# kjyv/FloBaRoID

Hardware: AMD Instinct MI355X
Metric: regressor samples/s (fused regressor->Gram pass) + TSQR TFLOP/s, WALK-MAN 31-DOF float-base (higher is better)
Workload: dtype f64

## Files before the change

flobaroid_amd/csrc/fbr_gram64.h:

```cpp
#pragma once
#define FBR_G64_SWZ(c) (2 * ((c) & 15))
#include <algorithm>
#include <type_traits>
#include <utility>

#include "fbr_kinid.h"

struct FbrGram64Tile {
    int col[FBR_TILE];
    std::vector<int> path;
    int friction = 0;
    int lo = 0, hi = 0;
};

struct FbrGram64 {
    int NT = 0;
    int NF = 0;
    int nlev = 0, fb = 0, flev = 0, ntr = 0, maxact = 0, npw = 0, wpb = 8;
    long blk_doubles = 0;
    std::vector<int> trow;
    std::vector<int> slab;
    int nstage = 0, base_stages = 0;
    std::vector<int> stage_lev;
    std::vector<int> lev_begin;
// ... 510 lines not shown
        const long grp = blk / bpg, lb = blk - grp * bpg;
        const long base = grp * Sg + (lb << 6);
        const int valid = (int)min(64L, Sg - (lb << 6));
        __syncthreads();
        {
            const long off = base * n;
            const int cnt = valid * n;
            int sr = tid / n, dc = tid - sr * n;
            const int ds = nth / n, dd = nth - ds * n;
            for (int i = tid; i < cnt; i += nth) {
                const double a = q[off + i], b = dq[off + i], c = ddq[off + i];
                sq[sr * ldn + dc] = a;
                sdq[sr * ldn + dc] = b;
                sddq[sr * ldn + dc] = c;
                sr += ds;
                dc += dd;
                if (dc >= n) {
                    dc -= n;
                    sr++;
                }
            }
            if (HASW || wr.k) {
                const int cw = valid * rows;
                int wr_ = tid / rows, wc = tid - wr_ * rows;
                const int es = nth / rows, ed = nth - es * rows;
                for (int i = tid; i < cw; i += nth) {
                    const double wv = HASW ? wts[base * rows + i] : 1.0;
                    if (HASW) sw[wr_ * ldw + wc] = wv;
                    if constexpr (KR == 1) {
                        if (wr.k) st[wr_ * ldw + wc] = wv * wv * rhs[base * rows + i];
                    } else {
#pragma unroll
                        for (int r = 0; r < KR; r++) st[r * 64 * ldw + wr_ * ldw + wc] = wv * wv * rhs[(base * rows + i) * KR + r];
                    }
                    wr_ += es;
                    wc += ed;
                    if (wc >= rows) {
                        wc -= rows;
                        wr_++;
                    }
                }
            }
        }
        __syncthreads();
        const int ls = min(lane, valid - 1);
        const long s = base + ls;
        const bool live = lane < valid;
        const double *mysq = sq + ls * ldn, *mysdq = sdq + ls * ldn, *mysddq = sddq + ls * ldn, *myw = sw + ls * ldw, *myt = st + ls * ldw;
        const long slot_off = blk * blk_doubles + (long)(lane >> 5) * 512;
        const int s31 = lane & 31;
        auto state = [&](int d, double &a, double &b, double &c) {
            a = mysq[d];
            b = mysdq[d];
            c = mysddq[d];
        };
        auto basest = [&](double *v6, double *a6, double *e3) {
            for (int i = 0; i < 6; i++) {
                v6[i] = bv[s * 6 + i];
                a6[i] = ba[s * 6 + i];
            }
            for (int i = 0; i < 3; i++) e3[i] = rpy[s * 3 + i];
        };
        auto save = [&](int b, int i, double v) { scr[(b * FBR_LINK_REC + i) * 64] = v; };
        auto load = [&](int b, int i) { return scr[(b * FBR_LINK_REC + i) * 64]; };
        auto consts = [&](int l, double *rR, double *rp, double *ax) {
            const fbr_cdouble_ptr cR = (fbr_cdouble_ptr)(unsigned long)m.restR, cp = (fbr_cdouble_ptr)(unsigned long)m.restp,
                                  ca = (fbr_cdouble_ptr)(unsigned long)m.axis;
            for (int i = 0; i < 9; i++) rR[i] = cR[9 * l + i];
            for (int i = 0; i < 3; i++) {
                rp[i] = cp[3 * l + i];
                ax[i] = ca[3 * l + i];
            }
        };
        const unsigned vlane = (unsigned)(((unsigned long)slot_off + (unsigned long)s31) << 3);
        auto link = [&](int l, int depth, const double *rec, const double (*Sst)[6], const int *lvd, double *F) {
            (void)F;
            if (wr.base_only) depth = 0;
            __builtin_amdgcn_s_waitcnt(0x0F70);
            long d10[10], dF[4];
#pragma unroll
            for (int pp = 0; pp < 10; pp++) d10[pp] = cdst[((long)part * m.L + l) * FBR_G64_WORDS + pp];
#pragma unroll
            for (int pp = 0; pp < 4; pp++) dF[pp] = cdst[((long)part * m.L + l) * FBR_G64_WORDS + 10 + pp];
            auto ft_of = [&](int ro, double *F) {
#pragma unroll
                for (int i = 0; i < 6; i++)
                    if (i < m.fb) F[i] = myt[ro + i];
#pragma unroll
                for (int j = 0; j < MAXD; j++)
                    if (j < depth) {
                        const double tj = myt[ro + m.fb + lvd[j]];
#pragma unroll
                        for (int i = 0; i < 6; i++) F[i] += Sst[j][i] * tj;
                    }
            };
            double Ft[6] = {0.0, 0.0, 0.0, 0.0, 0.0, 0.0};
            if constexpr (KR == 1) {
                if (wr.k) {
#pragma unroll
                    for (int i = 0; i < 6; i++)
                        if (i < m.fb) Ft[i] = myt[i];
#pragma unroll
                    for (int j = 0; j < MAXD; j++)
                        if (j < depth) {
                            const double tj = myt[m.fb + lvd[j]];
#pragma unroll
                            for (int i = 0; i < 6; i++) Ft[i] += Sst[j][i] * tj;
                        }
                }
            }
            auto ft_group = [&](int r, double *F) {
                int ro = r * 64 * ldw;
                asm volatile("" : "+v"(ro));
#pragma unroll
                for (int i = 0; i < 6; i++) F[i] = 0.0;
                ft_of(ro, F);
            };
            auto store = [&](long d0, int lv, double v) {
                if (d0 == 0) return;
                const unsigned vo = vlane ^ ((unsigned)(d0 & 0xff) << 3);
                __builtin_nontemporal_store(v, (fbr_gdouble_ptr)((fbr_gchar_ptr)(d0 & ~0xffL) + (long)lv * 8192 + vo));
            };
            auto full_group = [&](auto q0c, auto nqc) {
                constexpr int Q0 = decltype(q0c)::value, NQ = decltype(nqc)::value;
                double wA[NQ][6];
#pragma unroll
                for (int qq = 0; qq < NQ; qq++) fbr_unit_wrench(rec, Q0 + qq, wA[qq]);
#pragma unroll
                for (int i = 0; i < 6; i++)
                    if (i < m.fb) {
#pragma unroll
                        for (int qq = 0; qq < NQ; qq++) store(i < wr.flev ? dF[Q0 + qq] : d10[Q0 + qq], i, HASW ? wA[qq][i] * myw[i] : wA[qq][i]);
                    }
#pragma unroll
                for (int j = 0; j < MAXD; j++)
                    if (j < depth) {
                        double v[NQ];
#pragma unroll
                        for (int qq = 0; qq < NQ; qq++) v[qq] = fbr_dot6(Sst[j], wA[qq]);
                        const double wj = HASW ? myw[m.fb + lvd[j]] : 1.0;
#pragma unroll
                        for (int qq = 0; qq < NQ; qq++) store(d10[Q0 + qq], m.fb + j, HASW ? v[qq] * wj : v[qq]);
                    }
                if constexpr (KR == 1) {
                    if (wr.k) {
#pragma unroll
                        for (int qq = 0; qq < NQ; qq++)
                            if (d10[Q0 + qq]) unsafeAtomicAdd(mo + (long)ccol[10 * l + Q0 + qq] * 64 + lane, fbr_dot6(Ft, wA[qq]));
                    }
                } else {
#pragma unroll
                    for (int r = 0; r < KR; r++) {
                        double F[6];
                        ft_group(r, F);
#pragma unroll
                        for (int qq = 0; qq < NQ; qq++)
                            if (d10[Q0 + qq]) unsafeAtomicAdd(mo + ((long)r * wr.cols + ccol[10 * l + Q0 + qq]) * 64 + lane, fbr_dot6(F, wA[qq]));
                    }
                }
            };
            auto moment_group = [&](auto q0c, auto nqc) {
                constexpr int Q0 = decltype(q0c)::value, NQ = decltype(nqc)::value;
                double nB[NQ][3];
#pragma unroll
                for (int qq = 0; qq < NQ; qq++) fbr_unit_moment3(rec, 4 + Q0 + qq, nB[qq]);
#pragma unroll
                for (int i = 3; i < 6; i++)
                    if (i < m.fb) {
#pragma unroll
                        for (int qq = 0; qq < NQ; qq++) store(d10[4 + Q0 + qq], i, HASW ? nB[qq][i - 3] * myw[i] : nB[qq][i - 3]);
                    }
#pragma unroll
                for (int j = 0; j < MAXD; j++)
                    if (j < depth) {
                        double v[NQ];
#pragma unroll
                        for (int qq = 0; qq < NQ; qq++) v[qq] = Sst[j][3] * nB[qq][0] + Sst[j][4] * nB[qq][1] + Sst[j][5] * nB[qq][2];
                        const double wj = HASW ? myw[m.fb + lvd[j]] : 1.0;
#pragma unroll
                        for (int qq = 0; qq < NQ; qq++) store(d10[4 + Q0 + qq], m.fb + j, HASW ? v[qq] * wj : v[qq]);
                    }
                if constexpr (KR == 1) {
                    if (wr.k) {
#pragma unroll
                        for (int qq = 0; qq < NQ; qq++)
                            if (d10[4 + Q0 + qq])
                                unsafeAtomicAdd(mo + (long)ccol[10 * l + 4 + Q0 + qq] * 64 + lane, Ft[3] * nB[qq][0] + Ft[4] * nB[qq][1] + Ft[5] * nB[qq][2]);
                    }
                } else {
#pragma unroll
                    for (int r = 0; r < KR; r++) {
                        double F[6];
                        ft_group(r, F);
#pragma unroll
                        for (int qq = 0; qq < NQ; qq++)
                            if (d10[4 + Q0 + qq])
                                unsafeAtomicAdd(mo + ((long)r * wr.cols + ccol[10 * l + 4 + Q0 + qq]) * 64 + lane,
                                                F[3] * nB[qq][0] + F[4] * nB[qq][1] + F[5] * nB[qq][2]);
                    }
                }
            };
            using std::integral_constant;
            if constexpr (MAXD > 8 && MAXD <= 10) {
                full_group(integral_constant<int, 0>{}, integral_constant<int, 2>{});
                full_group(integral_constant<int, 2>{}, integral_constant<int, 2>{});
                moment_group(integral_constant<int, 0>{}, integral_constant<int, 3>{});
                moment_group(integral_constant<int, 3>{}, integral_constant<int, 3>{});
            } else {
                full_group(integral_constant<int, 0>{}, integral_constant<int, 4>{});
                moment_group(integral_constant<int, 0>{}, integral_constant<int, 6>{});
            }
            const int nfr = wr.cols > wr.ninert ? (wr.cols - wr.ninert) / n : 0;
            const int dj = nfr ? m.dof[l] : -1;
            if (dj >= 0 && depth > 0) {
                const fbr_cint_ptr cfr = (fbr_cint_ptr)(unsigned long)(wr.lcol10 + (long)wr.nparts * 10 * m.L + ((long)part * m.L + l) * FBR_G64_FRIC);
#pragma unroll
                for (int pf = 0; pf < FBR_G64_FRIC; pf++)
                    if (pf < nfr) {
                        const long dfw = cdst[((long)part * m.L + l) * FBR_G64_WORDS + 14 + pf];
                        if (dfw == 0) continue;
                        const int c = cfr[pf];
                        const double fv = fbr_friction_value(m.coldesc[c].z, mysdq[dj], sign ? sign[s * n + dj] : 0.0, m.stribeck);
                        store(dfw, m.fb + depth - 1, HASW ? fv * myw[m.fb + dj] : fv);
                        if constexpr (KR == 1) {
                            if (wr.k) unsafeAtomicAdd(mo + (long)c * 64 + lane, fv * myt[m.fb + dj]);
                        } else {
#pragma unroll
                            for (int r = 0; r < KR; r++) unsafeAtomicAdd(mo + ((long)r * wr.cols + c) * 64 + lane, fv * myt[r * 64 * ldw + m.fb + dj]);
                        }
                    }
            }
        };
        auto emit = [&](int, double) {};
        if (live) {
            fbr_kinid_lane<MAXD, false>(wr.part_nsteps[part], p.maxlvl, p.steps + wr.part_step0[part] * FBR_KINID_STEP, p.endflush, m.floating, m.g, m.fb,
                                        state, basest, save, load, link, emit, consts);
            if constexpr (KR == 1) {
                if (wr.k && part == wr.nparts - 1) {
                    double tt = 0.0;
                    for (int r = 0; r < rows; r++) {
                        const double wv = HASW ? myw[r] : 1.0, tv = rhs[s * rows + r] * wv;
                        tt += tv * tv;
                    }
                    unsafeAtomicAdd(mo + (long)wr.cols * 64 + lane, tt);
                }
            } else if (part == wr.nparts - 1) {
                double tt[KR * (KR + 1) / 2];
#pragma unroll
                for (int e = 0; e < KR * (KR + 1) / 2; e++) tt[e] = 0.0;
                for (int r = 0; r < rows; r++) {
                    const double wv = HASW ? myw[r] : 1.0;
                    double tv[KR];
#pragma unroll
                    for (int i = 0; i < KR; i++) tv[i] = rhs[(s * rows + r) * KR + i] * wv;
#pragma unroll
                    for (int i = 0, e = 0; i < KR; i++)
#pragma unroll
                        for (int j = i; j < KR; j++, e++) tt[e] += tv[i] * tv[j];
                }
#pragma unroll
                for (int e = 0; e < KR * (KR + 1) / 2; e++) unsafeAtomicAdd(mo + ((long)KR * wr.cols + e) * 64 + lane, tt[e]);
            }
        }
    }
}

__global__ __launch_bounds__(256) void fbr_gram64_tail_zero_kernel(double *__restrict__ img, long blk_doubles, long bpg, int ntr, int valid)
{
    double *blk = img + ((long)blockIdx.y * bpg + bpg - 1) * blk_doubles;
    const int per = 16 * (64 - valid);
    for (long e = (long)blockIdx.x * blockDim.x + threadIdx.x; e < (long)ntr * per; e += (long)gridDim.x * blockDim.x) {
        const int tr = (int)(e / per), r = (int)(e - (long)tr * per), c = r / (64 - valid), sl = valid + r % (64 - valid);
        blk[(long)tr * 1024 + (sl >> 5) * 512 + c * 32 + ((sl & 31) ^ FBR_G64_SWZ(c))] = 0.0;
    }
}

__global__ __launch_bounds__(256) void fbr_gram64_mom_reduce_kernel(int P, int k, int nwg, const double *__restrict__ mom, double *__restrict__ G)
{
    __shared__ double part[256];
    const int c = blockIdx.x, t = threadIdx.x, nm = fbr_gram64_mom_count(P, k);
    double s0 = 0.0, s1 = 0.0, s2 = 0.0, s3 = 0.0;
    int i = t;
    for (; i + 768 < nwg * 64; i += 1024) {
        s0 += mom[((long)(i >> 6) * nm + c) * 64 + (i & 63)];
        s1 += mom[((long)((i + 256) >> 6) * nm + c) * 64 + ((i + 256) & 63)];
        s2 += mom[((long)((i + 512) >> 6) * nm + c) * 64 + ((i + 512) & 63)];
        s3 += mom[((long)((i + 768) >> 6) * nm + c) * 64 + ((i + 768) & 63)];
    }
    for (; i < nwg * 64; i += 256) s0 += mom[((long)(i >> 6) * nm + c) * 64 + (i & 63)];
    part[t] = (s0 + s1) + (s2 + s3);
    __syncthreads();
    for (int o = 128; o > 0; o >>= 1) {
        if (t < o) part[t] += part[t + o];
        __syncthreads();
    }
    if (t) return;
    const int Pa = P + k;
    int row, col;
    fbr_gram64_mom_target(P, k, c, &row, &col);
    G[(long)row * Pa + col] += part[0];
    if (row != col) G[(long)col * Pa + row] += part[0];
}

template <int NPW, int WPB, bool RUNS = false>
__global__ __launch_bounds__(WPB * 64, (NPW <= 10) ? 4 : 2) void fbr_gram64_kernel(DevGram64 g, long nblk, const double *__restrict__ img,
                                                                                  double *__restrict__ partial, int carry)
{
    constexpr int MW = 3 * NPW;
    static_assert(MW <= 64, "a wave's slot table is fetched with one load");
    extern __shared__ __attribute__((aligned(16))) double smem[];
    const int bufd = g.maxact * 512;
    double *buf0 = smem, *buf1 = smem + bufd;
    int *slab = (int *)(smem + 2 * bufd);
    int *levb = slab + g.nlev * g.NT;
    int *pcs = levb + g.nlev + 1;
    int *wm = pcs + 2 * g.npieces;
    int *rn = wm + WPB * MW;
    static_assert(!RUNS || NPW > 10, "the 128-register shapes walk every slot");
    int *stl = rn + (RUNS ? WPB * g.nlev : 0);
    const int tid = threadIdx.x, lane = tid & 63;
    const int wave = __builtin_amdgcn_readfirstlane(tid >> 6);
    for (int i = tid; i < g.nlev * g.NT; i += WPB * 64) slab[i] = g.slab[i] * 512;
    for (int i = tid; i <= g.nlev; i += WPB * 64) levb[i] = g.lev_begin[i];
    for (int i = tid; i < 2 * g.npieces; i += WPB * 64) pcs[i] = g.pieces[i];
    for (int i = tid; i < WPB * MW; i += WPB * 64) wm[i] = g.wmeta[i];
    if (RUNS)
        for (int i = tid; i < WPB * g.nlev; i += WPB * 64) rn[i] = g.runs[i];
    for (int i = tid; i <= g.nstage; i += WPB * 64) stl[i] = g.stage_lev[i];
    fbr_d4 acc[NPW];
    img += (long)blockIdx.y * nblk * g.blk_doubles;
    double *pp = partial + (((((long)blockIdx.y * gridDim.x + blockIdx.x) * 8 + (wave & 7)) * (WPB / 8) + (wave >> 3)) * NPW) * 256;
    if (carry) {
#pragma unroll
        for (int q = 0; q < NPW; q++) acc[q] = (fbr_d4){pp[q * 256 + lane], pp[q * 256 + 64 + lane], pp[q * 256 + 128 + lane], pp[q * 256 + 192 + lane]};
    } else {
#pragma unroll
        for (int q = 0; q < NPW; q++) acc[q] = (fbr_d4){0.0, 0.0, 0.0, 0.0};
    }
    __syncthreads();
    const int nmine = (int)((nblk - blockIdx.x + gridDim.x - 1) / gridDim.x);
    const long nst = (long)(nmine > 0 ? nmine : 0) * 2 * g.nstage;
    const int svl = stl[lane <= g.nstage ? lane : 0], svp = levb[svl];
    auto dma = [&](int sg, long bh, int par) {
        const long blk = (long)blockIdx.x + (bh >> 1) * gridDim.x;
        const double *src = img + blk * g.blk_doubles + (bh & 1) * 512 + 2 * lane;
        double *buf = par ? buf1 : buf0;
        const int i0 = __builtin_amdgcn_readlane(svp, sg) + wave, i1 = __builtin_amdgcn_readlane(svp, sg + 1);
        const int mine = i0 < i1 ? (i1 - i0 + WPB - 1) / WPB : 0;
        const int il = i0 + (lane < mine ? lane : 0) * WPB;
        const int gxv = mine > 0 ? pcs[2 * il] : 0, lxv = mine > 0 ? pcs[2 * il + 1] : 0;
        for (int j = 0; j < mine; j++) {
            const int gx = __builtin_amdgcn_readlane(gxv, j), lx = __builtin_amdgcn_readlane(lxv, j);
            __builtin_amdgcn_global_load_lds((fbr_glb_ptr)(src + gx), (fbr_lds_ptr)(buf + lx), 16, 0, 0);
        }
    };
    if (nst > 0) dma(0, 0, 0);
    const int li = lane & 15, kk = lane >> 4;
    const int lofs = li * 32, sx = FBR_G64_SWZ(li);
    const int mv = wm[wave * MW + (lane < MW ? lane : 0)];
    const int idxv = (lane < MW && (lane % 3) != 2 && mv >= 0) ? mv : 0;
    const int p0c = lofs | (sx ^ kk);
    static_assert(!RUNS || MW < 63, "lane 63 holds the run");
    const int *lk = lane == 63 ? rn + wave * g.nlev : slab + idxv;
    const int lks = lane == 63 ? 1 : g.NT;
    const unsigned rlm = [&] {
        unsigned m = 0;
#pragma unroll
        for (int q = 1; q < NPW; q++) m |= (unsigned)(__builtin_amdgcn_readlane(mv, 3 * q) != __builtin_amdgcn_readlane(mv, 3 * q - 3)) << q;
        return (unsigned)__builtin_amdgcn_readfirstlane((int)m);
    }();
    int ko[8];
#pragma unroll
    for (int ks = 0; ks < 8; ks++) ko[ks] = (p0c ^ (4 * ks)) * 8;
    double X[2][8], Y[2][8];
#pragma unroll
    for (int ks = 0; ks < 8; ks++) X[0][ks] = X[1][ks] = Y[0][ks] = Y[1][ks] = 0.0;
    auto run_stage = [&](const double *buf, int lv0, int lv1) {
        const unsigned bufb = (unsigned)(unsigned long)(fbr_lds_ptr)buf;
        int offv = lk[lv0 * lks];
        for (int lv = lv0; lv < lv1; lv++) {
            const int cur = offv;
            offv = lk[(lv + 1 < g.nlev ? lv + 1 : lv) * lks];
            const int run = __builtin_amdgcn_readlane(cur, 63), qa = run & 0xff, qb = run >> 8;
#define G64_RD(D, S, K, T) "v_add_u32 %[" T "], %[" S "], %[o" #K "]\n\tds_read_b64 %[" D #K "], %[" T "]\n\t"
#define G64_MF(K) "v_mfma_f64_16x16x4_f64 %[acc], %[xa" #K "], %[xb" #K "], %[acc]\n\t"
#define G64_MV(K) "v_mov_b64 %[ya" #K "], %[xa" #K "]\n\t"
#pragma unroll
            for (int q = 0; q < NPW; q++) {
                if (q < qa || q >= qb) continue;
                const int P = q & 1, N = P ^ 1;
                int t0, t1;
                if (q == qa) {
                    const unsigned sa = bufb + (__builtin_amdgcn_readlane(cur, 3 * q) << 3), sb = bufb + (__builtin_amdgcn_readlane(cur, 3 * q + 1) << 3);
                    asm volatile(G64_RD("xa", "sa", 0, "t0") G64_RD("xa", "sa", 1, "t1") G64_RD("xa", "sa", 2, "t0") G64_RD("xa", "sa", 3, "t1")
                                 G64_RD("xa", "sa", 4, "t0") G64_RD("xa", "sa", 5, "t1") G64_RD("xa", "sa", 6, "t0") G64_RD("xa", "sa", 7, "t1")
                                 G64_RD("xb", "sb", 0, "t0") G64_RD("xb", "sb", 1, "t1") G64_RD("xb", "sb", 2, "t0") G64_RD("xb", "sb", 3, "t1")
                                 G64_RD("xb", "sb", 4, "t0") G64_RD("xb", "sb", 5, "t1") G64_RD("xb", "sb", 6, "t0") G64_RD("xb", "sb", 7, "t1")
                                 : [t0] "=&v"(t0), [t1] "=&v"(t1),
                                   [xa0] "+v"(X[P][0]), [xa1] "+v"(X[P][1]), [xa2] "+v"(X[P][2]), [xa3] "+v"(X[P][3]),
                                   [xa4] "+v"(X[P][4]), [xa5] "+v"(X[P][5]), [xa6] "+v"(X[P][6]), [xa7] "+v"(X[P][7]),
                                   [xb0] "+v"(Y[P][0]), [xb1] "+v"(Y[P][1]), [xb2] "+v"(Y[P][2]), [xb3] "+v"(Y[P][3]),
                                   [xb4] "+v"(Y[P][4]), [xb5] "+v"(Y[P][5]), [xb6] "+v"(Y[P][6]), [xb7] "+v"(Y[P][7])
                                 : [sa] "s"(sa), [sb] "s"(sb),
                                   [o0] "v"(ko[0]), [o1] "v"(ko[1]), [o2] "v"(ko[2]), [o3] "v"(ko[3]), [o4] "v"(ko[4]), [o5] "v"(ko[5]), [o6] "v"(ko[6]), [o7] "v"(ko[7])
                                 : "memory");
                }
                const int f = __builtin_amdgcn_readfirstlane((q + 1 < qb ? 4 : 0) | ((rlm >> (q + 1)) & 1 ? 8 : 0));
                const unsigned sna = q + 1 < NPW ? bufb + (__builtin_amdgcn_readlane(cur, 3 * q + 3) << 3) : 0u;
                const unsigned snb = q + 1 < NPW ? bufb + (__builtin_amdgcn_readlane(cur, 3 * q + 4) << 3) : 0u;
                asm volatile(
                    "s_waitcnt lgkmcnt(0)\n\t"
                    G64_MF(0)
                    "s_bitcmp0_b32 %[f], 2\n\t"
                    "s_cbranch_scc1 3f\n\t"
                    G64_RD("yb", "snb", 0, "t0") G64_RD("yb", "snb", 1, "t1") G64_MF(1)
                    G64_RD("yb", "snb", 2, "t0") G64_RD("yb", "snb", 3, "t1") G64_MF(2)
                    G64_RD("yb", "snb", 4, "t0") G64_RD("yb", "snb", 5, "t1") G64_MF(3)
                    G64_RD("yb", "snb", 6, "t0") G64_RD("yb", "snb", 7, "t1") G64_MF(4)
                    "s_bitcmp0_b32 %[f], 3\n\t"
                    "s_cbranch_scc1 2f\n\t"
                    G64_RD("ya", "sna", 0, "t0") G64_RD("ya", "sna", 1, "t1") G64_RD("ya", "sna", 2, "t0") G64_RD("ya", "sna", 3, "t1") G64_MF(5)
                    G64_RD("ya", "sna", 4, "t0") G64_RD("ya", "sna", 5, "t1") G64_RD("ya", "sna", 6, "t0") G64_RD("ya", "sna", 7, "t1") G64_MF(6)
                    G64_MF(7)
                    "s_branch 9f\n\t"
                    "2:\n\t"
                    G64_MV(0) G64_MV(1) G64_MV(2) G64_MV(3) G64_MF(5)
                    G64_MV(4) G64_MV(5) G64_MV(6) G64_MV(7) G64_MF(6)
                    G64_MF(7)
                    "s_branch 9f\n\t"
                    "3:\n\t"
                    G64_MF(1) G64_MF(2) G64_MF(3) G64_MF(4) G64_MF(5) G64_MF(6) G64_MF(7)
                    "9:"
                    : [acc] "+v"(acc[q]), [t0] "=&v"(t0), [t1] "=&v"(t1),
                      [xa0] "+v"(X[P][0]), [xa1] "+v"(X[P][1]), [xa2] "+v"(X[P][2]), [xa3] "+v"(X[P][3]),
                      [xa4] "+v"(X[P][4]), [xa5] "+v"(X[P][5]), [xa6] "+v"(X[P][6]), [xa7] "+v"(X[P][7]),
                      [xb0] "+v"(Y[P][0]), [xb1] "+v"(Y[P][1]), [xb2] "+v"(Y[P][2]), [xb3] "+v"(Y[P][3]),
                      [xb4] "+v"(Y[P][4]), [xb5] "+v"(Y[P][5]), [xb6] "+v"(Y[P][6]), [xb7] "+v"(Y[P][7]),
                      [ya0] "+v"(X[N][0]), [ya1] "+v"(X[N][1]), [ya2] "+v"(X[N][2]), [ya3] "+v"(X[N][3]),
                      [ya4] "+v"(X[N][4]), [ya5] "+v"(X[N][5]), [ya6] "+v"(X[N][6]), [ya7] "+v"(X[N][7]),
                      [yb0] "+v"(Y[N][0]), [yb1] "+v"(Y[N][1]), [yb2] "+v"(Y[N][2]), [yb3] "+v"(Y[N][3]),
                      [yb4] "+v"(Y[N][4]), [yb5] "+v"(Y[N][5]), [yb6] "+v"(Y[N][6]), [yb7] "+v"(Y[N][7])
                    : [f] "s"(f), [sna] "s"(sna), [snb] "s"(snb),
                      [o0] "v"(ko[0]), [o1] "v"(ko[1]), [o2] "v"(ko[2]), [o3] "v"(ko[3]), [o4] "v"(ko[4]), [o5] "v"(ko[5]), [o6] "v"(ko[6]), [o7] "v"(ko[7])
                    : "memory", "scc");
            }
#undef G64_RD
#undef G64_MF
#undef G64_MV
        }
    };
    int sg = 0;
    long bh = 0;
    for (long st = 0; st < nst; st++) {
        asm volatile("s_waitcnt vmcnt(0)" ::: "memory");
        __syncthreads();
        const int sgn = sg + 1 == g.nstage ? 0 : sg + 1;
        const long bhn = sgn ? bh : bh + 1;
        if (st + 1 < nst) dma(sgn, bhn, (int)((st + 1) & 1));
        const double *buf = (st & 1) ? buf1 : buf0;
        const int lv0 = __builtin_amdgcn_readlane(svl, sg), lv1 = __builtin_amdgcn_readlane(svl, sg + 1);
        sg = sgn;
        bh = bhn;
        if constexpr (RUNS) {
            run_stage(buf, lv0, lv1);
            continue;
        }
        for (int lv = lv0; lv < lv1; lv++) {
            const int offv = slab[lv * g.NT + idxv];
            int curI = -1;
            double a[8] = {0.0, 0.0, 0.0, 0.0, 0.0, 0.0, 0.0, 0.0};
#pragma unroll
            for (int q = 0; q < NPW; q++) {
                const int tI = __builtin_amdgcn_readlane(mv, 3 * q), rg = __builtin_amdgcn_readlane(mv, 3 * q + 2);
                if (tI < 0 || lv < (rg & 0xff) || lv >= (rg >> 8)) continue;
                const double *pb = buf + __builtin_amdgcn_readlane(offv, 3 * q + 1);
                double b[NPW <= 10 ? 4 : 8];
                int p0 = p0c;
                if constexpr (NPW <= 10) asm volatile("" : "+v"(p0));
                if (tI != curI) {
                    const double *pa = buf + __builtin_amdgcn_readlane(offv, 3 * q);
#pragma unroll
                    for (int ks = 0; ks < 8; ks++) a[ks] = pa[p0 ^ (4 * ks)];
                    curI = tI;
                }
                constexpr int KG = NPW <= 10 ? 4 : 8;
#pragma unroll
                for (int k0 = 0; k0 < 8; k0 += KG) {
#pragma unroll
                    for (int ks = k0; ks < k0 + KG; ks++) b[ks - k0] = pb[p0 ^ (4 * ks)];
                    __builtin_amdgcn_sched_barrier(0);
#pragma unroll
                    for (int ks = k0; ks < k0 + KG; ks++) acc[q] = __builtin_amdgcn_mfma_f64_16x16x4f64(a[ks], b[ks - k0], acc[q], 0, 0, 0);
                    __builtin_amdgcn_sched_barrier(0);
                }
            }
        }
    }
    if constexpr (RUNS) asm volatile("s_nop 7\n\ts_nop 7\n\ts_nop 7" ::: "memory");
#pragma unroll
    for (int q = 0; q < NPW; q++) {
        pp[q * 256 + 0 * 64 + lane] = acc[q][0];
        pp[q * 256 + 1 * 64 + lane] = acc[q][1];
        pp[q * 256 + 2 * 64 + lane] = acc[q][2];
        pp[q * 256 + 3 * 64 + lane] = acc[q][3];
    }
}
#endif
```

flobaroid_amd/csrc/fbr_gram_api.hip:

```cpp
#define FBR_KERNELS_GRAM
#include "fbr_internal.h"

static int get_deal(GramHolder *h, int wpg, GramHolder::Deal *out, bool base_only = false)
{
    const int key = wpg | (base_only ? 1 << 24 : 0);
    auto it = h->deals.find(key);
    if (it != h->deals.end()) {
        *out = it->second;
        return FBR_OK;
    }
    const std::vector<int> n = fbr_gram_deal(h->prog, wpg, base_only);
    std::vector<int2> tab;
    std::vector<int> begin(h->prog.T + 1, 0), given(h->prog.T, 0);
    for (int p = 0; p < h->prog.T; p++) begin[p + 1] = begin[p] + n[p];
    while ((int)tab.size() < begin[h->prog.T])
        for (int p = 0; p < h->prog.T; p++)
            if (given[p] < n[p]) tab.push_back(make_int2(p, given[p]++ | (n[p] << 16)));
    GramHolder::Deal d;
    int rc;
    if ((rc = upload(h->pool, tab, &d.tab))) return rc;
    if ((rc = upload(h->pool, begin, &d.begin))) return rc;
    h->deals[key] = d;
    *out = d;
    return FBR_OK;
// ... 663 lines not shown
            fresh_images = true;
        }
    HIPCHK(hipEventRecord(m->ev_fork, m->stream));
    hipStream_t side = m->opt.gram_serial ? m->stream : m->side;
    const bool cross = overlap_prev && !fresh_images && side != m->stream;
    if (!cross) HIPCHK(hipStreamWaitEvent(side, m->ev_fork, 0));
    if (h2d_chunked && (rc = ensure_stage_buffers(m, d, k, dw, ch, nchunks > 1 ? 2 : 1))) return rc;
    const int pack_wgs_per_cu = 24;
    const int pack_blocks_max = m->num_cus * pack_wgs_per_cu;
    auto produce = [&](long ci) -> int {
        const long s0 = items[ci].s0, cs = items[ci].cs;
        const int b = (int)(ci & 1);
        if (ci >= 2 || (cross && m->ev_gram_rec[b])) HIPCHK(hipStreamWaitEvent(side, m->ev_gram[b], 0));
        DevStates dc = d;
        long o = s0;
        const double *crhs = drhs, *cw = dw;
        if (h2d_chunked) {
            int r3;
            if ((r3 = ensure_copy_stream(m))) return r3;
            if (ci >= 2 || (cross && m->ev_pack_rec[b]))
                HIPCHK(hipStreamWaitEvent(m->copy, m->ev_pack[b], 0));
            else
                HIPCHK(hipStreamWaitEvent(m->copy, m->ev_fork, 0));
            ProfScope ps(m, FBR_PROF_H2D, m->copy);
            if ((r3 = stage_chunk(m, d, drhs, k, dw, s0, cs, b, m->copy, &dc, &crhs, &cw))) return r3;
            o = 0;
            HIPCHK(hipEventRecord(m->ev_h2d[b], m->copy));
            HIPCHK(hipStreamWaitEvent(side, m->ev_h2d[b], 0));
        }
        int rc2 = run_kin(m, dc, o, cs, side, &m->rec2);
        if (rc2) return rc2;
        {
            ProfScope ps(m, FBR_PROF_PACK, side);
            const int blocks = (int)std::min<long>(cs, (long)pack_blocks_max);
            hipLaunchKernelGGL(fbr_pack_kernel, dim3(blocks), dim3(256), h->pack_lds_bytes, side, h->dev, m->dm, cs, cs / items[ci].ng,
                               m->rec2.as<double>(), dc.dq + o * hm.n, dc.sign ? dc.sign + o * hm.n : nullptr,
                               crhs ? crhs + (size_t)o * hm.rows * k : nullptr, cw ? cw + (size_t)o * hm.rows : nullptr,
                               h->pimg[b].as<double>(), base_only ? 1 : 0, moments ? h->mom[(int)(m->next_ticket & 1)].as<double>() : nullptr);
        }
        HIPCHK(hipGetLastError());
        HIPCHK(hipEventRecord(m->ev_pack[b], side));
        m->ev_pack_rec[b] = true;
        return FBR_OK;
    };
    const int mpar = (int)(m->next_ticket & 1);
    if (moments) {
        const size_t mbytes = (size_t)pack_blocks_max * 256 * 4 * sizeof(double);
        if (h->mom[mpar].bytes < mbytes) h->mom_clean[mpar] = false;
        if ((rc = h->mom[mpar].ensure(mbytes))) return rc;
        if (!h->mom_clean[mpar]) HIPCHK(hipMemsetAsync(h->mom[mpar].p, 0, mbytes, side));
        h->mom_clean[mpar] = false;
    }
    if ((rc = produce(0))) return rc;
    for (long ci = 0; ci < nchunks; ci++) {
        const long cs = items[ci].cs;
        const int ng = items[ci].ng;
        const int b = (int)(ci & 1);
        if (ci + 1 < nchunks && (rc = produce(ci + 1))) return rc;
        HIPCHK(hipStreamWaitEvent(m->stream, m->ev_pack[b], 0));
        const int wpg = wpg_of(cs, ng);
        GramHolder::Deal deal;
        if ((rc = get_deal(h, wpg, &deal, base_only))) return rc;
        DevGram dg = h->dev;
        dg.wpg = wpg;
        dg.ks_limit = base_only ? hm.fbp / 4 : (1 << 20);
        if (base_only && hm.fbp == 8) {
            dg.pieces = dg.pieces_b;
            dg.piece_begin = dg.piece_begin_b;
        }
        dg.wg_tab = deal.tab;
        dg.wg_begin = deal.begin;
        const int NW = wpg * ng;
        const size_t pcount = (size_t)NW * FBR_WPB * FBR_NPW * 256;
        if ((rc = m->partial.ensure(pcount * sizeof(double)))) return rc;
        unsigned long long *dbg = nullptr;
        if (timing) {
            if ((rc = m->st_x.ensure((size_t)NW * FBR_WPB * 8 * sizeof(unsigned long long)))) return rc;
            dbg = m->st_x.as<unsigned long long>();
        }
        {
            ProfScope ps(m, FBR_PROF_GRAM);
            hipLaunchKernelGGL(gram_kernel, dim3(NW), dim3(FBR_WPB * 64), h->lds_bytes, m->stream, dg, cs, ng,
                               h->pimg[b].as<double>(), m->partial.as<double>(), dbg, (carry_ok && ci > 0) ? 1 : 0);
        }
        HIPCHK(hipGetLastError());
        HIPCHK(hipEventRecord(m->ev_gram[b], m->stream));
        m->ev_gram_rec[b] = true;
        if (timing && (rc = print_gram_timing(m, T, dbg, NW))) return rc;
        if (!carry_ok || ci + 1 == nchunks) {
            ProfScope ps(m, FBR_PROF_REDUCE);
            hipLaunchKernelGGL(fbr_gram_reduce_kernel, dim3(T * FBR_WPB * FBR_NPW, ng), dim3(256), 0, m->stream, dg,
                               m->partial.as<double>(), G + (size_t)items[ci].g0 * Pa * Pa);
        }
        HIPCHK(hipGetLastError());
    }
    if (moments) {
        ProfScope ps(m, FBR_PROF_REDUCE);
        hipLaunchKernelGGL(fbr_gram_mom_reduce_kernel, dim3(256), dim3(256), 0, m->stream, hm.cols, k, pack_blocks_max, h->itemcol,
                           h->mom[mpar].as<double>(), G);
        HIPCHK(hipGetLastError());
        h->mom_clean[mpar] = true;
    }
    if (!async) HIPCHK(hipStreamSynchronize(side));
    return FBR_OK;
}

static int gram_impl_inner(fbr_model *m, const fbr_states *st, const double *rhs, int32_t k, const double *w, double *G_out,
                           int32_t out_mem, int32_t accumulate, int32_t ngroups, int64_t *async_ticket)
{
    const bool async = async_ticket != nullptr;
    bool overlap_prev = false;
    const bool h2d_chunked = st && st->mem == FBR_HOST && m && m->opt.h2d_chunked && is_pinned_host(st->q) && is_pinned_host(st->dq) &&
                             is_pinned_host(st->ddq) && is_pinned_host(st->base_vel) && is_pinned_host(st->base_acc) &&
                             is_pinned_host(st->base_rpy) && is_pinned_host(st->sign) && is_pinned_host(rhs) && is_pinned_host(w);
    if (async && (!st || out_mem != FBR_DEVICE || (st->mem != FBR_DEVICE && !h2d_chunked))) {
        set_err("fbr_gram_submit takes a device-resident output and device-resident or PINNED host states / rhs / weights");
        return FBR_E_INVALID;
    }
    DevStates d;
    if (m) m->submitting = async;
    int rc = stage_states(m, st, &d, true, h2d_chunked);
    if (m) m->submitting = false;
    if (rc) return rc;
    if (async) {
        if ((rc = wait_ticket(m, m->next_ticket - 2))) return rc;
        overlap_prev = m->waited_ticket < m->next_ticket - 1;
    }
    if (!G_out || k < 0 || k > FBR_MAX_RHS || (k > 0 && !rhs)) {
        set_err("bad rhs / G_out arguments");
        return FBR_E_INVALID;
    }
    if (ngroups < 1 || d.S % ngroups != 0) {
        set_err("the number of samples must be a multiple of the number of groups");
        return FBR_E_INVALID;
    }
    const FbrHostModel &hm = m->hm;
    if ((hm.rows + 3) / 4 * 4 > 60) {
        if (async || ngroups != 1) {
            set_err("robots with more than 60 regressor rows per sample (54 DOF on a floating base) are served by the blocking, ungrouped "
                    "fbr_gram_accumulate only (Gram from the TSQR factor): fbr_gram_submit / fbr_gram_grouped are limited to 60 rows");
            return FBR_E_UNSUPPORTED;
        }
        return gram_via_tsqr(m, st, rhs, k, w, G_out, out_mem, accumulate);
    }
    GramHolder *h = nullptr;
    const bool moments = ngroups == 1 && fbr_gram_rhs_moments(hm, k, m->opt.gram_rhs_tile != 0) && !m->opt.gram_timing;
    if ((rc = get_gram(m, k, &h, moments))) return rc;
    const int Pa = h->prog.Pa;
    const size_t gcount = (size_t)Pa * Pa * ngroups;
    const long S = d.S;
    const double *drhs = nullptr, *dw = nullptr;
    if (h2d_chunked) {
        drhs = rhs;
        dw = w;
    } else {
        if ((rc = stage_one(m, m->st_aux, rhs, (size_t)S * hm.rows * k, st->mem, &drhs))) return rc;
        if ((rc = stage_one(m, m->st_aux2, w, (size_t)S * hm.rows, st->mem, &dw))) return rc;
    }
    bool base_only = false;
    if (w && S > 0 && hm.fb > 0 && hm.rows > hm.fb) {
        if (st->mem == FBR_HOST) {
            base_only = true;
            for (long s = 0; s < S && base_only; s++)
                for (int r = hm.fb; r < hm.rows; r++)
                    if (w[s * hm.rows + r] != 0.0) {
                        base_only = false;
                        break;
                    }
        } else {
            std::vector<char> act;
            if ((rc = active_rows(m, dw, S, &act))) return rc;
            base_only = true;
            for (int r = hm.fb; r < hm.rows; r++) base_only = base_only && !act[r];
        }
    }
    double *G = G_out;
    if (out_mem == FBR_HOST) {
        if ((rc = m->g_tmp.ensure(gcount * sizeof(double)))) return rc;
        G = m->g_tmp.as<double>();
        if (accumulate) HIPCHK(hipMemcpyAsync(G, G_out, gcount * sizeof(double), hipMemcpyHostToDevice, m->stream));
    }
    if (!accumulate) HIPCHK(hipMemsetAsync(G, 0, gcount * sizeof(double), m->stream));
    bool lane = false;
    if (S > 0 && d.q && !m->opt.gram_timing && !m->opt.gram_serial && (ngroups == 1 || (k == 0 && !h2d_chunked && !base_only)) &&
        (rc = gram64_serves(m, h, k, &lane)))
        return rc;
    if (lane && ngroups > 1 && (S / ngroups + 63) / 64 <= gram64_chunk_blocks(h->g64))
        rc = gram64_grouped_pass(m, h, d, dw, G, ngroups);
    else if (lane && ngroups == 1)
        rc = gram64_pass(m, h, d, drhs, dw, k, G, base_only && h->g64.base_stages > 0, h2d_chunked);
    else if (S > 0)
        rc = gram_image_pass(m, h, d, drhs, dw, k, G, ngroups, base_only, h2d_chunked, overlap_prev, async);
    if (rc) return rc;
    if (S > 0 && !async && h2d_chunked && m->copy) HIPCHK(hipStreamSynchronize(m->copy));
    if (async) {
        const int64_t t = m->next_ticket++;
        m->ticket_kind[t & 1] = 0;
        m->last_submit_kind = 0;
        HIPCHK(hipEventRecord(m->ev_done[t & 1], m->stream));
        *async_ticket = t;
        return FBR_OK;
    }
    return finish_output(m, G, G_out, gcount, out_mem);
}

static int gram_impl(fbr_model *m, const fbr_states *st, const double *rhs, int32_t k, const double *w, double *G_out, int32_t out_mem,
                     int32_t accumulate, int32_t ngroups, int64_t *async_ticket);

static int gram_via_red(fbr_model *m, int which, const fbr_states *st, const double *rhs, int32_t k, const double *w, double *G_out, int32_t out_mem,
                        int32_t accumulate, int32_t ngroups, int64_t *async_ticket)
{
    fbr_model *r = m->rdm[which].get();
    const bool async = async_ticket != nullptr;
    int rc;
    if ((rc = enter(m))) return rc;
    if ((rc = wait_ticket(m, async ? m->next_ticket - 2 : m->next_ticket - 1))) return rc;
    if (async && out_mem != FBR_DEVICE) {
        set_err("fbr_gram_submit takes a device-resident output and device-resident or PINNED host states / rhs / weights");
        return FBR_E_INVALID;
    }
    r->stream = m->stream;
    r->prof = m->prof;
    const int par = (int)(m->next_ticket & 1), Pa = m->hm.cols + k, Pra = r->hm.cols + k;
    if (ngroups < 1 || (async && ngroups != 1)) {
        set_err("bad number of groups");
        return FBR_E_INVALID;
    }
    const size_t cnt = (size_t)Pa * Pa * ngroups;
    if ((rc = m->red_out[par].ensure((size_t)Pra * Pra * ngroups * sizeof(double)))) return rc;
    double *Gred = m->red_out[par].as<double>();
    int64_t tr = -1;
    if ((rc = gram_impl(r, st, rhs, k, w, Gred, FBR_DEVICE, 0, ngroups, async ? &tr : nullptr))) return rc;
    double *G = G_out;
    if (out_mem == FBR_HOST) {
        if ((rc = m->g_tmp.ensure(cnt * sizeof(double)))) return rc;
        G = m->g_tmp.as<double>();
        if (accumulate) HIPCHK(hipMemcpyAsync(G, G_out, cnt * sizeof(double), hipMemcpyHostToDevice, m->stream));
    }
    if ((rc = m->red_w.ensure((size_t)Pra * Pa * ngroups * sizeof(double)))) return rc;
    for (int g0 = 0; g0 < ngroups; g0 += 32768) {
        const int ng = std::min(32768, ngroups - g0);
        hipLaunchKernelGGL(fbr_expand_rows_kernel, dim3(ng > 1 ? 64 : 512, ng), dim3(256), 0, m->stream, m->hm.cols, k, Pra, m->E_beg[which], m->E_row[which],
                           m->E_val[which], Gred + (size_t)g0 * Pra * Pra, m->red_w.as<double>() + (size_t)g0 * Pra * Pa, Pa, (const int *)nullptr, Pa);
        hipLaunchKernelGGL(fbr_expand_gram_kernel, dim3(ng > 1 ? 128 : 1024, ng), dim3(256), 0, m->stream, m->hm.cols, k, Pra, m->E_beg[which], m->E_row[which],
                           m->E_val[which], m->red_w.as<double>() + (size_t)g0 * Pra * Pa, G + (size_t)g0 * Pa * Pa, accumulate ? 1 : 0);
    }
    HIPCHK(hipGetLastError());
    if (async) {
        const int64_t t = m->next_ticket++;
        m->ticket_kind[t & 1] = 0;
        m->ticket_via_red[t & 1] = 1 + which;
        m->red_ticket[t & 1] = tr;
        m->last_submit_kind = 0;
        HIPCHK(hipEventRecord(m->ev_done[t & 1], m->stream));
        *async_ticket = t;
        return FBR_OK;
    }
    return finish_output(m, G, G_out, cnt, out_mem);
}

static int gram_impl(fbr_model *m, const fbr_states *st, const double *rhs, int32_t k, const double *w, double *G_out,
                     int32_t out_mem, int32_t accumulate, int32_t ngroups, int64_t *async_ticket = nullptr)
{
    const bool grouped_ok = st && (ngroups == 1 || (ngroups >= 1 && (double)(st->num_samples / ngroups) >= m->opt.reduce_grouped_min_samples));
    const int which =
        (m && st && ngroups >= 1 && G_out && k >= 0 && k <= FBR_MAX_RHS && m->pid == getpid() && grouped_ok) ? pick_gram_reduction(m, (long)st->num_samples) : -1;
    if (which >= 0) {
        int rc = gram_via_red(m, which, st, rhs, k, w, G_out, out_mem, accumulate, ngroups, async_ticket);
        if (rc && m->stream) {
            const std::string msg = g_fbr_err;
            drain_after_failed_submit(m);
            set_err(msg);
        }
        return rc;
    }
    int rc = gram_impl_inner(m, st, rhs, k, w, G_out, out_mem, accumulate, ngroups, async_ticket);
    if (rc && m && m->pid == getpid() && m->stream) {
        const std::string msg = g_fbr_err;
        drain_after_failed_submit(m);
        set_err(msg);
    }
    return rc;
}
extern "C" int fbr_gram_accumulate(fbr_model *m, const fbr_states *st, const double *rhs, int32_t k, const double *w,
                                   double *G_out, int32_t out_mem, int32_t accumulate)
{
    return gram_impl(m, st, rhs, k, w, G_out, out_mem, accumulate, 1);
}

extern "C" int fbr_gram_submit(fbr_model *m, const fbr_states *st, const double *rhs, int32_t k, const double *w, double *G_out,
                               int32_t accumulate, int64_t *ticket)
{
    if (!ticket) {
        set_err("ticket is NULL");
        return FBR_E_INVALID;
    }
    return gram_impl(m, st, rhs, k, w, G_out, FBR_DEVICE, accumulate, 1, ticket);
}
extern "C" int fbr_gram_grouped(fbr_model *m, const fbr_states *st, int32_t ngroups, const double *rhs, int32_t k, const double *w,
                                double *G_out, int32_t out_mem)
{
    return gram_impl(m, st, rhs, k, w, G_out, out_mem, 0, ngroups);
}
```

Baseline: 85.76 million.

## Defer next-stage DMA issue into the MFMA loop for RUNS kernel

For the RUNS variant, the next stage's global-to-LDS DMA is no longer issued right after the barrier. Its addresses are computed one stage ahead and the loads are issued after the first slot's LDS reads inside the level loop, so they overlap with MFMA work. The offset prefetch now carries across stages and wraps at the last level instead of being reloaded per stage. It also adds optional, compile-time-gated s_memtime phase instrumentation and a host API to read it back. The wrap-around offset load and the staging parity logic add a risk of subtle indexing errors.

```diff
diff --git a/flobaroid_amd/csrc/fbr_gram64.h b/flobaroid_amd/csrc/fbr_gram64.h
--- a/flobaroid_amd/csrc/fbr_gram64.h
+++ b/flobaroid_amd/csrc/fbr_gram64.h
@@ -836,6 +836,14 @@
     if (row != col) G[(long)col * Pa + row] += part[0];
 }
 
+#ifdef FBR_G64_PHASES
+#define FBR_G64_PH_WGS 256
+__device__ unsigned long long fbr_g64_phase_buf[FBR_G64_PH_WGS * 8 * 8];
+#define G64_PH(...) __VA_ARGS__
+#else
+#define G64_PH(...)
+#endif
+
 template <int NPW, int WPB, bool RUNS = false>
 __global__ __launch_bounds__(WPB * 64, (NPW <= 10) ? 4 : 2) void fbr_gram64_kernel(DevGram64 g, long nblk, const double *__restrict__ img,
                                                                                   double *__restrict__ partial, int carry)
@@ -888,7 +896,29 @@
             __builtin_amdgcn_global_load_lds((fbr_glb_ptr)(src + gx), (fbr_lds_ptr)(buf + lx), 16, 0, 0);
         }
     };
-    if (nst > 0) dma(0, 0, 0);
+    int dma_n = 0, dma_gx = 0, dma_lx = 0, dma_par = 0;
+    long dma_bh = 0;
+    auto dma_fetch = [&](int sg, long bh, int par) {
+        const int i0 = __builtin_amdgcn_readlane(svp, sg) + wave, i1 = __builtin_amdgcn_readlane(svp, sg + 1);
+        dma_n = i0 < i1 ? (i1 - i0 + WPB - 1) / WPB : 0;
+        const int il = i0 + (lane < dma_n ? lane : 0) * WPB;
+        dma_gx = dma_n > 0 ? pcs[2 * il] : 0, dma_lx = dma_n > 0 ? pcs[2 * il + 1] : 0;
+        dma_bh = bh, dma_par = par;
+    };
+    auto dma_issue = [&]() {
+        const long blk = (long)blockIdx.x + (dma_bh >> 1) * gridDim.x;
+        const double *src = img + blk * g.blk_doubles + (dma_bh & 1) * 512 + 2 * lane;
+        double *buf = dma_par ? buf1 : buf0;
+        for (int j = 0; j < dma_n; j++) {
+            const int gx = __builtin_amdgcn_readlane(dma_gx, j), lx = __builtin_amdgcn_readlane(dma_lx, j);
+            __builtin_amdgcn_global_load_lds((fbr_glb_ptr)(src + gx), (fbr_lds_ptr)(buf + lx), 16, 0, 0);
+        }
+        dma_n = 0;
+    };
+    if (nst > 0) {
+        dma(0, 0, 0);
+        if (RUNS && nst > 1) dma_fetch(g.nstage > 1 ? 1 : 0, g.nstage > 1 ? 0 : 1, 1);
+    }
     const int li = lane & 15, kk = lane >> 4;
     const int lofs = li * 32, sx = FBR_G64_SWZ(li);
     const int mv = wm[wave * MW + (lane < MW ? lane : 0)];
@@ -909,12 +939,15 @@
     double X[2][8], Y[2][8];
 #pragma unroll
     for (int ks = 0; ks < 8; ks++) X[0][ks] = X[1][ks] = Y[0][ks] = Y[1][ks] = 0.0;
+    G64_PH(unsigned long long ph[8] = {0, 0, 0, 0, 0, 0, 0, 0}, ph_mark = 0; int ph_open = 0;)
+    const int lvend = __builtin_amdgcn_readlane(svl, g.nstage);
+    int offv = lk[0];
     auto run_stage = [&](const double *buf, int lv0, int lv1) {
         const unsigned bufb = (unsigned)(unsigned long)(fbr_lds_ptr)buf;
-        int offv = lk[lv0 * lks];
         for (int lv = lv0; lv < lv1; lv++) {
+            G64_PH(if (!ph_open) ph_mark = __builtin_amdgcn_s_memtime();)
             const int cur = offv;
-            offv = lk[(lv + 1 < g.nlev ? lv + 1 : lv) * lks];
+            offv = lk[(lv + 1 < lvend ? lv + 1 : 0) * lks];
             const int run = __builtin_amdgcn_readlane(cur, 63), qa = run & 0xff, qb = run >> 8;
 #define G64_RD(D, S, K, T) "v_add_u32 %[" T "], %[" S "], %[o" #K "]\n\tds_read_b64 %[" D #K "], %[" T "]\n\t"
 #define G64_MF(K) "v_mfma_f64_16x16x4_f64 %[acc], %[xa" #K "], %[xb" #K "], %[acc]\n\t"
@@ -938,6 +971,8 @@
                                  : [sa] "s"(sa), [sb] "s"(sb),
                                    [o0] "v"(ko[0]), [o1] "v"(ko[1]), [o2] "v"(ko[2]), [o3] "v"(ko[3]), [o4] "v"(ko[4]), [o5] "v"(ko[5]), [o6] "v"(ko[6]), [o7] "v"(ko[7])
                                  : "memory");
+                    G64_PH(asm volatile("s_waitcnt lgkmcnt(0)" ::: "memory"); ph[ph_open ? 3 : 4] += __builtin_amdgcn_s_memtime() - ph_mark;
+                           ph[6] += ph_open ? 0 : 1; ph_open = 0;)
                 }
                 const int f = __builtin_amdgcn_readfirstlane((q + 1 < qb ? 4 : 0) | ((rlm >> (q + 1)) & 1 ? 8 : 0));
                 const unsigned sna = q + 1 < NPW ? bufb + (__builtin_amdgcn_readlane(cur, 3 * q + 3) << 3) : 0u;
@@ -977,6 +1012,7 @@
                     : [f] "s"(f), [sna] "s"(sna), [snb] "s"(snb),
                       [o0] "v"(ko[0]), [o1] "v"(ko[1]), [o2] "v"(ko[2]), [o3] "v"(ko[3]), [o4] "v"(ko[4]), [o5] "v"(ko[5]), [o6] "v"(ko[6]), [o7] "v"(ko[7])
                     : "memory", "scc");
+                if (q == qa && dma_n > 0) dma_issue();
             }
 #undef G64_RD
 #undef G64_MF
@@ -985,18 +1021,28 @@
     };
     int sg = 0;
     long bh = 0;
+    G64_PH(const unsigned long long ph_begin = __builtin_amdgcn_s_memtime();)
     for (long st = 0; st < nst; st++) {
+        G64_PH(const unsigned long long ph_t0 = __builtin_amdgcn_s_memtime();)
         asm volatile("s_waitcnt vmcnt(0)" ::: "memory");
+        G64_PH(const unsigned long long ph_t1 = __builtin_amdgcn_s_memtime();)
         __syncthreads();
+        G64_PH(if (ph_open) ph[3] += ph_t0 - ph_mark;
+               ph_mark = __builtin_amdgcn_s_memtime(); ph_open = 1; ph[1] += ph_t1 - ph_t0; ph[2] += ph_mark - ph_t1; ph[5] += 1;)
         const int sgn = sg + 1 == g.nstage ? 0 : sg + 1;
         const long bhn = sgn ? bh : bh + 1;
-        if (st + 1 < nst) dma(sgn, bhn, (int)((st + 1) & 1));
+        if constexpr (!RUNS) {
+            if (st + 1 < nst) dma(sgn, bhn, (int)((st + 1) & 1));
+        }
         const double *buf = (st & 1) ? buf1 : buf0;
         const int lv0 = __builtin_amdgcn_readlane(svl, sg), lv1 = __builtin_amdgcn_readlane(svl, sg + 1);
         sg = sgn;
         bh = bhn;
         if constexpr (RUNS) {
             run_stage(buf, lv0, lv1);
+            if (dma_n > 0) dma_issue();
+            const int sg2 = sgn + 1 == g.nstage ? 0 : sgn + 1;
+            if (st + 2 < nst) dma_fetch(sg2, sg2 ? bhn : bhn + 1, (int)(st & 1));
             continue;
         }
         for (int lv = lv0; lv < lv1; lv++) {
@@ -1031,6 +1077,18 @@
         }
     }
     if constexpr (RUNS) asm volatile("s_nop 7\n\ts_nop 7\n\ts_nop 7" ::: "memory");
+    G64_PH(if (RUNS && blockIdx.y == 0 && blockIdx.x < FBR_G64_PH_WGS) {
+        const unsigned long long ph_end = __builtin_amdgcn_s_memtime();
+        if (ph_open) ph[3] += ph_end - ph_mark;
+        ph[0] = ph_end - ph_begin;
+        const unsigned long long ph_c = __builtin_amdgcn_s_memtime();
+        ph[7] = __builtin_amdgcn_s_memtime() - ph_c;
+        if (lane < 8) {
+            unsigned long long v = 0;
+            for (int i = 0; i < 8; i++) v = lane == i ? ph[i] : v;
+            fbr_g64_phase_buf[(blockIdx.x * 8 + (wave & 7)) * 8 + lane] += v;
+        }
+    })
 #pragma unroll
     for (int q = 0; q < NPW; q++) {
         pp[q * 256 + 0 * 64 + lane] = acc[q][0];
diff --git a/flobaroid_amd/csrc/fbr_gram_api.hip b/flobaroid_amd/csrc/fbr_gram_api.hip
--- a/flobaroid_amd/csrc/fbr_gram_api.hip
+++ b/flobaroid_amd/csrc/fbr_gram_api.hip
@@ -989,3 +989,17 @@
 {
     return gram_impl(m, st, rhs, k, w, G_out, out_mem, 0, ngroups);
 }
+
+#ifdef FBR_G64_PHASES
+extern "C" int fbr_gram64_phases(unsigned long long *out, int32_t reset)
+{
+    HIPCHK(hipDeviceSynchronize());
+    if (out) HIPCHK(hipMemcpyFromSymbol(out, HIP_SYMBOL(fbr_g64_phase_buf), sizeof(unsigned long long) * FBR_G64_PH_WGS * 64));
+    if (reset) {
+        void *p = nullptr;
+        HIPCHK(hipGetSymbolAddress(&p, HIP_SYMBOL(fbr_g64_phase_buf)));
+        HIPCHK(hipMemset(p, 0, sizeof(unsigned long long) * FBR_G64_PH_WGS * 64));
+    }
+    return FBR_OK;
+}
+#endif
```

After: 85.07 million. About the same (-0.8%).
